# gaspachoo/EEG2Video

Measured on AMD Instinct MI355X. Metric: 6-frame 288x512 clips/sec (50-step DDIM), higher is better.
Workload: dtype f32; 1 GPU; 1xMI355X: batch=8/GPU synthetic latents [B,4,6,36,64] + [B,77,768] cond, 50-step DDIM, CFG 12.5, 288x512x6 VAE decode, fp32 (BASELINE configs[1]); clips_per_gpu=8, ddim_steps=50, unet_samples_per_ddim_step=16, weights=random-init SD-v1-4 architecture, counter RNG seed 42/43, collective=none

## Files before the change

### eeg2video_amd/csrc/attn.hip

```cpp
#include "h16.h"
#include "kernels.h"
#include "prof.h"
#include "runtime.h"
#include "act_io.h"

#include <cstdlib>
#include <type_traits>

namespace e2v {

typedef float f32x16 __attribute__((ext_vector_type(16)));
typedef float f32x4 __attribute__((ext_vector_type(4)));

struct AttnBlock { int qb, head, sf; bool valid; };
__host__ __device__ __forceinline__ int attn_xcd_unit(const int n, const int F, const int heads) {
    return n % 8 == 0 ? 0 : (n * F) % 8 == 0 ? 1 : 2;
}
__device__ __forceinline__ AttnBlock attn_block_of(const AttnArgs& p, const int nqb) {
    const int b = blockIdx.x, xcd = b & 7, idx = b >> 3;
    const int S = p.n * p.F;
    const int unit = attn_xcd_unit(p.n, p.F, p.heads);
    AttnBlock r;
    if (unit == 0) {
        const int per = p.F * p.heads * nqb;
        const int ul = idx / per, w = idx - ul * per;
        const int smp = ul * 8 + xcd;
        const int f = w / (p.heads * nqb), w2 = w - f * (p.heads * nqb);
        r.sf = smp * p.F + f; r.head = w2 / nqb; r.qb = w2 - r.head * nqb; r.valid = smp < p.n;
    } else if (unit == 1) {
        const int per = p.heads * nqb;
        const int ul = idx / per, w = idx - ul * per;
        r.sf = ul * 8 + xcd; r.head = w / nqb; r.qb = w - r.head * nqb; r.valid = r.sf < S;
    } else {
        const int ul = idx / nqb;
        const int pair = ul * 8 + xcd;
        r.qb = idx - ul * nqb; r.sf = pair / p.heads; r.head = pair - r.sf * p.heads; r.valid = pair < S * p.heads;
    }
    return r;
}
__device__ __forceinline__ AttnBlock attn_block(const AttnArgs& p) { return attn_block_of(p, (p.Nq + 127) / 128); }
static inline unsigned attn_grid_of(const AttnArgs& a, const unsigned nqb) {
    const int unit = attn_xcd_unit(a.n, a.F, a.heads);
    if (unit == 0) return 8u * (a.n / 8) * (unsigned)(a.F * a.heads) * nqb;
    if (unit == 1) return 8u * ((a.n * a.F) / 8) * (unsigned)a.heads * nqb;
    return 8u * ((a.n * a.F * a.heads + 7) / 8) * nqb;
}
static inline unsigned attn_grid(const AttnArgs& a) { return attn_grid_of(a, (a.Nq + 127) / 128); }

std::string attn_shape_tag(const AttnArgs& a) {
    return " D" + std::to_string(a.D) + " Nq" + std::to_string(a.Nq) + " Nk" + std::to_string(a.Nk) + " n" + std::to_string(a.n) + " F" + std::to_string(a.F) +
           " h" + std::to_string(a.heads);
}

template <int D>
__global__ __launch_bounds__(256) void flash_attn_kernel(const AttnArgs p) {
    constexpr int LD = D + 4;
    constexpr int TF = D / 32;
    constexpr bool VREM = (D - 32 * TF) == 8;
    constexpr int T = VREM ? TF : (D + 31) / 32;
    constexpr int TA = T > 0 ? T : 1;
    constexpr int G = D / 8;
    constexpr int DQ = D / 4;
    constexpr int KT = 32;
    constexpr int NF4 = KT * DQ;
    constexpr int LPT = (NF4 + 255) / 256;
    extern __shared__ __attribute__((aligned(16))) float smem[];

    const int tid = threadIdx.x;
    const int lane = tid & 63, wave = tid >> 6;
    const int j = lane & 31, h = lane >> 5;
    const AttnBlock blk = attn_block(p);
    if (!blk.valid) return;
    const int sf = blk.sf;
    const int smp = sf / p.F, f = sf - smp * p.F;
    const int head = blk.head;
    const int q0 = (blk.qb * 4 + wave) * 32;
    const bool active = q0 < p.Nq;

    int nseg = 1;
    size_t kvbase[2];
    if (p.mode == 0) {
        kvbase[0] = (size_t)(smp * p.F) * p.Nk;
        kvbase[1] = (size_t)(smp * p.F + (f > 0 ? f - 1 : 0)) * p.Nk;
        nseg = f >= 2 ? 2 : 1;
    } else {
        kvbase[0] = kvbase[1] = (size_t)smp * p.Nk;
    }
    const int tps = (p.Nk + KT - 1) / KT;
    const int ntiles = nseg * tps;

    f32x4 qf[G];
    {
        const int qrow = min(q0 + j, p.Nq - 1);
        const float* qp = p.q + ((size_t)sf * p.Nq + qrow) * p.ldq + head * D + h * 4;
        const float c = p.scale * 1.44269504088896340736f;
#pragma unroll
        for (int g = 0; g < G; ++g) {
            qf[g] = *reinterpret_cast<const f32x4*>(qp + g * 8);
            qf[g] *= c;
        }
    }

    constexpr unsigned OOB = 0x80000000u;
    auto rsrc_of = [](const void* ptr) {
        const unsigned long long v = reinterpret_cast<unsigned long long>(ptr);
        const unsigned lo = __builtin_amdgcn_readfirstlane((unsigned)v);
        const unsigned hi = __builtin_amdgcn_readfirstlane((unsigned)(v >> 32));
        return __builtin_amdgcn_make_buffer_rsrc(reinterpret_cast<void*>(((unsigned long long)hi << 32) | lo), (short)0, 0x7FFFFFF0,
                                                 0x00020000);
    };
    int ld_row[LPT];
    unsigned ld_off[LPT];
#pragma unroll
    for (int e = 0; e < LPT; ++e) {
        const int idx = tid + 256 * e;
        const int row = idx / DQ, c4 = idx - row * DQ;
        ld_row[e] = row;
        ld_off[e] = idx < NF4 ? (unsigned)(row * p.ldkv + c4 * 4) * 4u : OOB;
    }
    f32x4 kreg[LPT], vreg[LPT];
    auto load_tile = [&](int tt) {
        const int seg = tt / tps;
        const int key0 = (tt - seg * tps) * KT;
        const size_t first = (kvbase[seg] + key0) * p.ldkv + head * D;
        const __amdgpu_buffer_rsrc_t rk = rsrc_of(p.k + first), rv = rsrc_of(p.v + first);
        const int left = p.Nk - key0;
#pragma unroll
        for (int e = 0; e < LPT; ++e) {
            unsigned off = ld_off[e];
            if (left < KT) off = ld_row[e] < left ? off : OOB;
            kreg[e] = __builtin_bit_cast(f32x4, __builtin_amdgcn_raw_buffer_load_b128(rk, off, 0, 0));
            vreg[e] = __builtin_bit_cast(f32x4, __builtin_amdgcn_raw_buffer_load_b128(rv, off, 0, 0));
        }
    };
    auto store_tile = [&](int buf) {
        float* Ks = smem + buf * (2 * KT * LD);
        float* Vs = Ks + KT * LD;
#pragma unroll
        for (int e = 0; e < LPT; ++e) {
            const int idx = tid + 256 * e;
            if (idx < NF4) {
                const int row = idx / DQ, c4 = idx - row * DQ;
                *reinterpret_cast<f32x4*>(Ks + row * LD + c4 * 4) = kreg[e];
                *reinterpret_cast<f32x4*>(Vs + row * LD + c4 * 4) = vreg[e];
            }
        }
    };

    f32x16 acc[TA];
#pragma unroll
    for (int t = 0; t < TA; ++t)
#pragma unroll
        for (int r = 0; r < 16; ++r) acc[t][r] = 0.f;
    f32x4 rem0 = {0.f, 0.f, 0.f, 0.f}, rem1 = {0.f, 0.f, 0.f, 0.f};
    float m_i = -INFINITY, l_i = 0.f;

    load_tile(0);
    store_tile(0);
    __syncthreads();

    for (int tt = 0; tt < ntiles; ++tt) {
        const int buf = tt & 1;
        if (tt + 1 < ntiles) load_tile(tt + 1);
        const int seg_c = tt / tps;
        const int kbase = (tt - seg_c * tps) * KT;
        auto tile_body = [&](const int key0, const int sub, auto ragged) {
            const float* Ks = smem + buf * (2 * KT * LD) + sub * 32 * LD;
            const float* Vs = smem + buf * (2 * KT * LD) + KT * LD + sub * 32 * LD;
            const f32x16 zero16 = {0.f, 0.f, 0.f, 0.f, 0.f, 0.f, 0.f, 0.f, 0.f, 0.f, 0.f, 0.f, 0.f, 0.f, 0.f, 0.f};
            f32x16 st;
            const float* kp = Ks + j * LD + h * 4;
#pragma unroll
            for (int g = 0; g < G; ++g) {
                const f32x4 kf = *reinterpret_cast<const f32x4*>(kp + g * 8);
#pragma unroll
                for (int s = 0; s < 4; ++s)
                    st = __builtin_amdgcn_mfma_f32_32x32x2f32(kf[s], qf[g][s], (g == 0 && s == 0) ? zero16 : st, 0, 0, 0);
            }
            if constexpr (decltype(ragged)::value) {
#pragma unroll
                for (int r = 0; r < 16; ++r) {
                    const int key = key0 + (r & 3) + 8 * (r >> 2) + 4 * h;
                    if (key >= p.Nk) st[r] = -INFINITY;
                }
            }
            float mt = st[0];
#pragma unroll
            for (int r = 1; r < 16; ++r) mt = __builtin_fmaxf(mt, st[r]);
            mt = __builtin_fmaxf(mt, __shfl_xor(mt, 32));
            const float m_new = __builtin_fmaxf(m_i, mt);
            const bool moved = __any(m_new > m_i);
            float ps = 0.f;
#pragma unroll
            for (int r = 0; r < 16; ++r) {
                st[r] = __builtin_amdgcn_exp2f(st[r] - m_new);
                ps += st[r];
            }
            float alpha = 1.0f;
            if (moved) {
                alpha = __builtin_amdgcn_exp2f(m_i - m_new);
                l_i *= alpha;
            }
            l_i += ps;
            m_i = m_new;
#pragma unroll
            for (int t = 0; t < T; ++t) {
                if (moved) {
#pragma unroll
                    for (int r = 0; r < 16; ++r) acc[t][r] *= alpha;
                }
                const int dv = min(t * 32 + j, D - 1);
                const float* vp = Vs + (4 * h) * LD + dv;
#pragma unroll
                for (int r = 0; r < 16; ++r) {
                    const float vv = vp[((r & 3) + 8 * (r >> 2)) * LD];
                    acc[t] = __builtin_amdgcn_mfma_f32_32x32x2f32(vv, st[r], acc[t], 0, 0, 0);
                }
            }
            if constexpr (VREM) {
                if (moved) {
                    rem0 *= alpha;
                    rem1 *= alpha;
                }
                const float* vr = Vs + (4 * h) * LD + 32 * TF;
#pragma unroll
                for (int r = 0; r < 16; ++r) {
                    const float* row = vr + ((r & 3) + 8 * (r >> 2)) * LD;
                    const f32x4 v0 = *reinterpret_cast<const f32x4*>(row);
                    const f32x4 v1 = *reinterpret_cast<const f32x4*>(row + 4);
                    rem0 += v0 * st[r];
                    rem1 += v1 * st[r];
                }
            }
        };
#pragma unroll
        for (int sub = 0; sub < KT / 32; ++sub) {
            const int key0 = kbase + 32 * sub;
            if (active && key0 < p.Nk) {
                if (key0 + 32 <= p.Nk) tile_body(key0, sub, std::false_type{});
                else tile_body(key0, sub, std::true_type{});
            }
        }
        if (tt + 1 < ntiles) store_tile(buf ^ 1);
        __syncthreads();
    }

    const float l_tot = l_i + __shfl_xor(l_i, 32);
    if constexpr (VREM) {
#pragma unroll
        for (int e = 0; e < 4; ++e) {
            rem0[e] += __shfl_xor(rem0[e], 32);
            rem1[e] += __shfl_xor(rem1[e], 32);
        }
    }
    if (active && q0 + j < p.Nq) {
        const float inv = 1.0f / l_tot;
        float* op = p.o + ((size_t)sf * p.Nq + q0 + j) * p.ldo + head * D;
#pragma unroll
        for (int t = 0; t < T; ++t)
#pragma unroll
            for (int rg = 0; rg < 4; ++rg) {
                const int dv = t * 32 + 8 * rg + 4 * h;
                if (dv < D) {
                    f32x4 o;
#pragma unroll
                    for (int e = 0; e < 4; ++e) o[e] = acc[t][rg * 4 + e] * inv;
                    *reinterpret_cast<f32x4*>(op + dv) = o;
                }
            }
        if constexpr (VREM) {
            const f32x4 o = (h ? rem1 : rem0) * inv;
            *reinterpret_cast<f32x4*>(op + 32 * TF + 4 * h) = o;
        }
    }
}

typedef __bf16 abf16x4 __attribute__((ext_vector_type(4)));
typedef __bf16 abf16x8 __attribute__((ext_vector_type(8)));

template <typename H, int D, bool FOLD, int KT>
__global__ __launch_bounds__(256) void flash_attn_b16io_kernel(const AttnArgs p) {
    constexpr int DP = (D + 15) / 16 * 16;
    constexpr int KS = DP / 16;
    constexpr int T = (D + 31) / 32;
    constexpr int KROW = DP * 2 + 16;
    constexpr int VROW = ((T * 16) % 32 == 16) ? T * 64 : T * 64 + 64;
    constexpr int KBYTES = KT * KROW, VBYTES = KT * VROW;
    constexpr int STAGE = (KBYTES + VBYTES + 15) / 16 * 16;
    constexpr bool SUMV = (D % 32) != 0;
    constexpr int LROW = D % 32, LREG = 4 * (LROW / 8) + (LROW & 3), LHALF = (LROW >> 2) & 1;
    constexpr int C8 = D / 8;
    constexpr int NP = KT * C8;
    constexpr int LPT = (NP + 255) / 256;
    extern __shared__ __attribute__((aligned(16))) char smem_h[];

    const int tid = threadIdx.x;
    const int lane = tid & 63, wave = tid >> 6;
    const int j = lane & 31, h = lane >> 5;
    const AttnBlock blk = attn_block(p);
    if (!blk.valid) return;
    const int sf = blk.sf;
    const int smp = sf / p.F, f = sf - smp * p.F;
    const int head = blk.head;
    const int q0 = (blk.qb * 4 + wave) * 32;
    const bool active = q0 < p.Nq;
    const H* __restrict__ Q = reinterpret_cast<const H*>(p.q);
    const H* __restrict__ K = reinterpret_cast<const H*>(p.k);
    const H* __restrict__ V = reinterpret_cast<const H*>(p.v);

    int nseg = 1;
    size_t kvbase[2];
    if (p.mode == 0) {
        kvbase[0] = (size_t)(smp * p.F) * p.Nk;
        kvbase[1] = (size_t)(smp * p.F + (f > 0 ? f - 1 : 0)) * p.Nk;
        nseg = f >= 2 ? 2 : 1;
    } else {
        kvbase[0] = kvbase[1] = (size_t)smp * p.Nk;
    }
    const int tps = (p.Nk + KT - 1) / KT;
    const int ntiles = nseg * tps;

    for (int i = tid * 16; i < 2 * STAGE; i += 256 * 16)
        *reinterpret_cast<f32x4*>(smem_h + i) = f32x4{0.f, 0.f, 0.f, 0.f};
    if constexpr (SUMV) {
        __syncthreads();
        if (tid < 2 * KT)
            *reinterpret_cast<H*>(smem_h + (tid / KT) * STAGE + KBYTES + (tid % KT) * VROW + D * 2) = (H)1.0f;
    }

    hx8<H> qf[KS];
    {
        const int qrow = min(q0 + j, p.Nq - 1);
        const H* qp = Q + ((size_t)sf * p.Nq + qrow) * p.ldq + head * D;
#pragma unroll
        for (int s = 0; s < KS; ++s) {
            const int k0 = 16 * s + 8 * h;
            hx8<H> a;
#pragma unroll
            for (int e = 0; e < 8; ++e) a[e] = (H)0.f;
            if (k0 < D) a = *reinterpret_cast<const hx8<H>*>(qp + k0);
            if constexpr (FOLD) {
                const float qs = p.scale * 1.44269504088896340736f;
#pragma unroll
                for (int e = 0; e < 8; ++e) a[e] = (H)((float)a[e] * qs);
            }
            qf[s] = a;
        }
    }
    const float sc = p.scale * 1.44269504088896340736f;
    __syncthreads();

    constexpr unsigned OOB = 0x80000000u;
    auto rsrc_of = [](const void* ptr) {
        const unsigned long long v = reinterpret_cast<unsigned long long>(ptr);
        const unsigned lo = __builtin_amdgcn_readfirstlane((unsigned)v);
        const unsigned hi = __builtin_amdgcn_readfirstlane((unsigned)(v >> 32));
        return __builtin_amdgcn_make_buffer_rsrc(reinterpret_cast<void*>(((unsigned long long)hi << 32) | lo), (short)0, 0x7FFFFFF0,
                                                 0x00020000);
    };
    int ld_row[LPT], ld_c8[LPT];
    unsigned ld_off[LPT];
#pragma unroll
    for (int e = 0; e < LPT; ++e) {
        const int idx = tid + 256 * e;
        const int row = idx / C8, c8 = idx - row * C8;
        ld_row[e] = row; ld_c8[e] = c8;
        ld_off[e] = idx < NP ? (unsigned)(row * p.ldkv + c8 * 8) * 2u : OOB;
    }
    f32x4 kreg[LPT], vreg[LPT];
    auto load_tile = [&](const int seg, const int key0) {
        const size_t first = (kvbase[seg] + key0) * p.ldkv + head * D;
        const __amdgpu_buffer_rsrc_t rk = rsrc_of(K + first), rv = rsrc_of(V + first);
        const int left = p.Nk - key0;
#pragma unroll
        for (int e = 0; e < LPT; ++e) {
            unsigned off = ld_off[e];
            if (left < KT) off = ld_row[e] < left ? off : OOB;
            kreg[e] = __builtin_bit_cast(f32x4, __builtin_amdgcn_raw_buffer_load_b128(rk, off, 0, 0));
            vreg[e] = __builtin_bit_cast(f32x4, __builtin_amdgcn_raw_buffer_load_b128(rv, off, 0, 0));
        }
    };
    auto store_tile = [&](int buf) {
        char* Kl = smem_h + buf * STAGE;
        char* Vl = Kl + KBYTES;
#pragma unroll
        for (int e = 0; e < LPT; ++e) {
            if (tid + 256 * e < NP) {
                *reinterpret_cast<f32x4*>(Kl + ld_row[e] * KROW + ld_c8[e] * 16) = kreg[e];
                *reinterpret_cast<f32x4*>(Vl + ld_row[e] * VROW + ld_c8[e] * 16) = vreg[e];
            }
        }
    };

    f32x16 acc[T];
#pragma unroll
    for (int t = 0; t < T; ++t)
#pragma unroll
        for (int r = 0; r < 16; ++r) acc[t][r] = 0.f;
// ... 495 lines not shown
                for (int x = 0; x < 4; ++x) {
                    unsigned v1, v2, v3;
                    split3(vreg[e][x], v1, v2, v3);
                    char* vd = Vl + (c4 * 4 + x) * VROW + row * 2;
                    *reinterpret_cast<unsigned short*>(vd) = (unsigned short)(v1 >> 16);
                    *reinterpret_cast<unsigned short*>(vd + VBYTES) = (unsigned short)(v2 >> 16);
                    *reinterpret_cast<unsigned short*>(vd + 2 * VBYTES) = (unsigned short)(v3 >> 16);
                }
            }
        }
    };

    f32x16 acc[T];
#pragma unroll
    for (int t = 0; t < T; ++t)
#pragma unroll
        for (int r = 0; r < 16; ++r) acc[t][r] = 0.f;
    float m_i = -INFINITY, l_i = 0.f;

    load_tile(0);
    store_tile(0);
    __syncthreads();

    constexpr int TA[6] = {1, 2, 0, 1, 0, 0}, TB[6] = {1, 0, 2, 0, 1, 0};
    for (int tt = 0; tt < ntiles; ++tt) {
        const int buf = tt & 1;
        if (tt + 1 < ntiles) load_tile(tt + 1);
        const int seg_c = tt / tps;
        const int key0 = (tt - seg_c * tps) * 32;
        if (active) {
            const char* Kl = smem_x + buf * STAGE;
            const char* Vl = Kl + 3 * KBYTES;
            f32x16 st;
#pragma unroll
            for (int r = 0; r < 16; ++r) st[r] = 0.f;
            const char* kp = Kl + j * KROW + h * 16;
#pragma unroll
            for (int s = 0; s < KS; ++s) {
                abf16x8 kf[3];
#pragma unroll
                for (int pl = 0; pl < 3; ++pl) kf[pl] = *reinterpret_cast<const abf16x8*>(kp + pl * KBYTES + s * 32);
#pragma unroll
                for (int t6 = 0; t6 < 6; ++t6)
                    st = __builtin_amdgcn_mfma_f32_32x32x16_bf16(kf[TA[t6]], __builtin_bit_cast(abf16x8, qf[TB[t6]][s]), st, 0, 0, 0);
            }
            if (key0 + 32 > p.Nk) {
#pragma unroll
                for (int r = 0; r < 16; ++r) {
                    const int key = key0 + (r & 3) + 8 * (r >> 2) + 4 * h;
                    if (key >= p.Nk) st[r] = -INFINITY;
                }
            }
            float mt = st[0];
#pragma unroll
            for (int r = 1; r < 16; ++r) mt = __builtin_fmaxf(mt, st[r]);
            mt = __builtin_fmaxf(mt, __shfl_xor(mt, 32));
            const float m_new = __builtin_fmaxf(m_i, mt);
            const bool moved = __any(m_new > m_i);
            float ps = 0.f;
#pragma unroll
            for (int r = 0; r < 16; ++r) {
                st[r] = __builtin_amdgcn_exp2f(st[r] - m_new);
                ps += st[r];
            }
            float alpha = 1.0f;
            if (moved) {
                alpha = __builtin_amdgcn_exp2f(m_i - m_new);
                l_i *= alpha;
            }
            l_i += ps;
            m_i = m_new;
            au32x4 pf[3][2];
#pragma unroll
            for (int s = 0; s < 2; ++s)
#pragma unroll
                for (int e = 0; e < 4; ++e) {
                    unsigned a1, a2, a3, b1, b2, b3;
                    split3(st[8 * s + 2 * e], a1, a2, a3);
                    split3(st[8 * s + 2 * e + 1], b1, b2, b3);
                    pf[0][s][e] = (a1 >> 16) | (b1 & 0xFFFF0000u);
                    pf[1][s][e] = (a2 >> 16) | (b2 & 0xFFFF0000u);
                    pf[2][s][e] = (a3 >> 16) | (b3 & 0xFFFF0000u);
                }
#pragma unroll
            for (int t = 0; t < T; ++t) {
                if (moved) {
#pragma unroll
                    for (int r = 0; r < 16; ++r) acc[t][r] *= alpha;
                }
                const char* vrow = Vl + min(t * 32 + j, D - 1) * VROW + h * 8;
#pragma unroll
                for (int s = 0; s < 2; ++s) {
                    abf16x8 vf[3];
#pragma unroll
                    for (int pl = 0; pl < 3; ++pl) {
                        const abf16x4 lo = *reinterpret_cast<const abf16x4*>(vrow + pl * VBYTES + s * 32);
                        const abf16x4 hi = *reinterpret_cast<const abf16x4*>(vrow + pl * VBYTES + s * 32 + 16);
                        vf[pl] = __builtin_shufflevector(lo, hi, 0, 1, 2, 3, 4, 5, 6, 7);
                    }
#pragma unroll
                    for (int t6 = 0; t6 < 6; ++t6)
                        acc[t] = __builtin_amdgcn_mfma_f32_32x32x16_bf16(vf[TA[t6]], __builtin_bit_cast(abf16x8, pf[TB[t6]][s]), acc[t], 0, 0, 0);
                }
            }
        }
        if (tt + 1 < ntiles) store_tile(buf ^ 1);
        __syncthreads();
    }

    const float l_tot = l_i + __shfl_xor(l_i, 32);
    if (active && q0 + j < p.Nq) {
        const float inv = 1.0f / l_tot;
        float* op = p.o + ((size_t)sf * p.Nq + q0 + j) * p.ldo + head * D;
#pragma unroll
        for (int t = 0; t < T; ++t)
#pragma unroll
            for (int rg = 0; rg < 4; ++rg) {
                const int dv = t * 32 + 8 * rg + 4 * h;
                if (dv < D) {
                    f32x4 o;
#pragma unroll
                    for (int e = 0; e < 4; ++e) o[e] = acc[t][rg * 4 + e] * inv;
                    *reinterpret_cast<f32x4*>(op + dv) = o;
                }
            }
    }
}
template <int D>
static void launch_flash_x3(const AttnArgs& a, hipStream_t s) {
    constexpr int DP = (D + 15) / 16 * 16;
    constexpr size_t stage = ((size_t)3 * (32 * (DP * 2 + 16) + ((D + 31) / 32) * 32 * 72) + 15) / 16 * 16;
    constexpr size_t smem = 2 * stage;
    E2V_KATTR(&flash_attn_x3_kernel<D>, smem);
    dim3 grid(attn_grid(a), 1, 1);
    const double nk = a.mode == 0 ? 2.0 * a.Nk : (double)a.Nk;
    const double probs = (double)a.n * a.F * a.heads;
    ProfScope ps(a.mode == 0 ? "flash_attn_f32x3_sparse_causal" : "flash_attn_f32x3_cross", 4.0 * probs * a.Nq * nk * D,
                 4.0 * probs * D * (2.0 * a.Nq + 2.0 * (a.mode == 0 ? a.Nk : (double)a.Nk / a.F)), s);
    E2V_KLAUNCH((flash_attn_x3_kernel<D>), grid, dim3(256), smem, s, a);
}

template <int D>
static void launch_flash(const AttnArgs& a, hipStream_t s) {
    constexpr size_t smem = (size_t)2 * 2 * 32 * (D + 4) * sizeof(float);
    E2V_KATTR(&flash_attn_kernel<D>, smem);
    dim3 grid(attn_grid(a), 1, 1);
    const double nk = a.mode == 0 ? 2.0 * a.Nk : (double)a.Nk;
    const double probs = (double)a.n * a.F * a.heads;
    std::string pname = a.mode == 0 ? "flash_attn_sparse_causal" : "flash_attn_cross";
    if (prof_detail()) pname += attn_shape_tag(a);
    ProfScope ps(pname.c_str(), 4.0 * probs * a.Nq * nk * D,
                 4.0 * probs * D * (2.0 * a.Nq + 2.0 * (a.mode == 0 ? a.Nk : (double)a.Nk / a.F)), s);
    dry_tag(" -> flash_attn_kernel");
    E2V_KLAUNCH((flash_attn_kernel<D>), grid, dim3(256), smem, s, a);
}

bool flash_attention_supports(int D) {
    switch (D) {
        case 8: case 16: case 32: case 40: case 64: case 80: case 160: return true;
        default: return false;
    }
}

void flash_attention(const AttnArgs& a, hipStream_t s) {
    if (!flash_attention_supports(a.D))
        throw Error(E2V_EINVAL, "attention head dim " + std::to_string(a.D) + " has no kernel instance (supported: 8, 16, 32, 40, 64, 80, 160)");
    if (a.io_bf16) {
        if ((a.ldq | a.ldkv | a.ldo) & 7) throw Error(E2V_ESHAPE, "bf16 attention: row strides must be multiples of 8 elements");
        switch (a.D) {
            case 8: launch_flash_b16io<8>(a, s); return;
            case 16: launch_flash_b16io<16>(a, s); return;
            case 32: launch_flash_b16io<32>(a, s); return;
            case 40: launch_flash_b16io<40>(a, s); return;
            case 64: launch_flash_b16io<64>(a, s); return;
            case 80: launch_flash_b16io<80>(a, s); return;
            default: launch_flash_b16io<160>(a, s); return;
        }
    }
    if (a.x3) {
        switch (a.D) {
            case 8: launch_flash_x3<8>(a, s); return;
            case 16: launch_flash_x3<16>(a, s); return;
            case 32: launch_flash_x3<32>(a, s); return;
            case 40: launch_flash_x3<40>(a, s); return;
            case 64: launch_flash_x3<64>(a, s); return;
            case 80: launch_flash_x3<80>(a, s); return;
            default: launch_flash_x3<160>(a, s); return;
        }
    }
    switch (a.D) {
        case 8: launch_flash<8>(a, s); break;
        case 16: launch_flash<16>(a, s); break;
        case 32: launch_flash<32>(a, s); break;
        case 40: launch_flash<40>(a, s); break;
        case 64: launch_flash<64>(a, s); break;
        case 80: launch_flash<80>(a, s); break;
        default: launch_flash<160>(a, s); break;
    }
}

static constexpr int FMAX = 8;
template <typename T>
__global__ __launch_bounds__(256) void temporal_attn_kernel(const T* __restrict__ qkv, int ld, T* __restrict__ out,
                                                            int ldo, int n, int F, int HW, int heads, int D, float scale) {
    const size_t total = (size_t)n * HW * heads * F;
    const size_t gid = blockIdx.x * (size_t)blockDim.x + threadIdx.x;
    if (gid >= total) return;
    const int i = gid % F;
    const int head = (gid / F) % heads;
    const size_t ph = gid / ((size_t)F * heads);
    const int pix = ph % HW;
    const int smp = ph / HW;
    const int C = heads * D;
    const size_t row0 = (size_t)smp * F * HW + pix;
    const T* qp = qkv + (row0 + (size_t)i * HW) * ld + head * D;
    const T* kp = qkv + row0 * ld + C + head * D;
    const T* vp = qkv + row0 * ld + 2 * C + head * D;
    const size_t fstride = (size_t)HW * ld;
    float s[FMAX];
#pragma unroll
    for (int jf = 0; jf < FMAX; ++jf) s[jf] = 0.f;
    for (int c = 0; c < D; c += 4) {
        const f32x4 qv = ld4(qp + c);
#pragma unroll
        for (int jf = 0; jf < FMAX; ++jf)
            if (jf < F) {
                const f32x4 kv = ld4(kp + jf * fstride + c);
                s[jf] += qv[0] * kv[0] + qv[1] * kv[1] + qv[2] * kv[2] + qv[3] * kv[3];
            }
    }
    float m = -INFINITY;
#pragma unroll
    for (int jf = 0; jf < FMAX; ++jf)
        if (jf < F) {
            s[jf] *= scale;
            m = fmaxf(m, s[jf]);
        }
    float l = 0.f;
#pragma unroll
    for (int jf = 0; jf < FMAX; ++jf)
        if (jf < F) {
            s[jf] = expf(s[jf] - m);
            l += s[jf];
        }
    const float inv = 1.0f / l;
    T* op = out + (row0 + (size_t)i * HW) * ldo + head * D;
    for (int c = 0; c < D; c += 4) {
        f32x4 o = {0.f, 0.f, 0.f, 0.f};
#pragma unroll
        for (int jf = 0; jf < FMAX; ++jf)
            if (jf < F) {
                const f32x4 vv = ld4(vp + jf * fstride + c);
                o += vv * (s[jf] * inv);
            }
        st4(op + c, o);
    }
}

template <typename T>
__global__ __launch_bounds__(128) void temporal_attn_lds_kernel(const T* __restrict__ qkv, int ld, T* __restrict__ out,
                                                                int ldo, int F, int HW, int C, int D, float scale, int PB,
                                                                int CS, int npg) {
    extern __shared__ __attribute__((aligned(16))) float sm[];
    const int smp = blockIdx.x / npg, p0 = (blockIdx.x - smp * npg) * PB;
    const int c_base = blockIdx.y * CS;
    if constexpr (!std::is_same<T, float>::value) {
        const int CO = CS / 8;
        const int total = F * PB * 3 * CO;
        for (int idx = threadIdx.x; idx < total; idx += 128) {
            const int c8 = idx % CO;
            int r = idx / CO;
            const int part = r % 3; r /= 3;
            const int pp = r % PB;
            const int f = r / PB;
            const int pix = p0 + pp;
            f32x4 lo = {0.f, 0.f, 0.f, 0.f}, hi = lo;
            if (pix < HW) {
                const hx8<T> v = *reinterpret_cast<const hx8<T>*>(qkv + ((size_t)(smp * F + f) * HW + pix) * ld + part * C + c_base + c8 * 8);
#pragma unroll
                for (int e = 0; e < 4; ++e) { lo[e] = (float)v[e]; hi[e] = (float)v[4 + e]; }
            }
            *reinterpret_cast<f32x4*>(sm + (size_t)idx * 8) = lo;
            *reinterpret_cast<f32x4*>(sm + (size_t)idx * 8 + 4) = hi;
        }
    } else {
        const int CQ = CS / 4;
        const int total = F * PB * 3 * CQ;
        for (int idx = threadIdx.x; idx < total; idx += 128) {
            const int c4 = idx % CQ;
            int r = idx / CQ;
            const int part = r % 3; r /= 3;
            const int pp = r % PB;
            const int f = r / PB;
            const int pix = p0 + pp;
            f32x4 v = {0.f, 0.f, 0.f, 0.f};
            if (pix < HW) v = ld4(qkv + ((size_t)(smp * F + f) * HW + pix) * ld + part * C + c_base + c4 * 4);
            *reinterpret_cast<f32x4*>(sm + (size_t)idx * 4) = v;
        }
    }
    __syncthreads();
    const int hs = CS / D;
    const int items = PB * hs * F;
    for (int item = threadIdx.x; item < items; item += 128) {
        const int i = item % F;
        const int hh = (item / F) % hs;
        const int pp = item / (F * hs);
// ... 495 lines not shown
```

### eeg2video_amd/csrc/bgemm.hip

```cpp
#include "igemm_epi.h"
#include "prof.h"
#include "runtime.h"

#include <cstdio>
#include <cstdlib>
#include <string>

#include <map>
#include <mutex>

namespace e2v {

static std::mutex& knob_mutex() { static std::mutex m; return m; }
static std::map<std::string, int>& knob_table() { static std::map<std::string, int> t; return t; }
int* knob(const char* name, int dflt) {
    std::lock_guard<std::mutex> lk(knob_mutex());
    auto& t = knob_table();
    auto it = t.find(name);
    if (it == t.end()) {
        const char* e = std::getenv(name);
        it = t.emplace(name, e ? std::atoi(e) : dflt).first;
    }
    return &it->second;
}
bool set_knob(const char* name, int value) {
    std::lock_guard<std::mutex> lk(knob_mutex());
    auto& t = knob_table();
    auto it = t.find(name);
    if (it == t.end()) {
        static const char* const known[] = {"E2V_BGEMM_PERS", "E2V_BGEMM_256LIN", "E2V_BGEMM_256", "E2V_BGEMM_T256", "E2V_BGEMM_T256P", "E2V_BGEMM_T256P_BIAS_LDS",
                                            "E2V_ATTN_KT64", "E2V_ATTN_Q64", "E2V_ATTN_CROSS_RESIDENT", "E2V_TATTN_WAVE", "E2V_LN_ROWS", "E2V_BGEMM_UP2X",
                                            "E2V_SPLITK", "E2V_SPLITK_FORCE", "E2V_GN_FUSED_SMALL", "E2V_BGEMM_S3_SMALL", "E2V_SMALL_FAMILY_CLIPS", "E2V_POOL_GUARD"
#ifdef E2V_AB
                                            , "E2V_BGEMM_S3", "E2V_BGEMM_LIN", "E2V_BGEMM_T256_TAIL", "E2V_ATTN_FOLD", "E2V_ATTN_Q64P", "E2V_ATTN_Q64_NW", "E2V_GN_ROWS", "E2V_GN_GROUP_MB", "E2V_GN_SKIP_PARTIAL", "E2V_GN_RB", "E2V_GN_RB_EPILOGUE",
                                            "E2V_BGEMM_256_MINROUNDS", "E2V_BGEMM_T256_MINK", "E2V_BGEMM_T256_MINTILES", "E2V_BGEMM_T256P_MAXK", "E2V_BGEMM_T256P_MINTILES", "E2V_GN_CHUNK_ROWS",
                                            "E2V_GN_CHUNK_ROWS_SMALL", "E2V_IGEMM_HALF_BELOW", "E2V_SPLITK_MIN_DEPTH", "E2V_SPLITK_MAX_TILES", "E2V_GN_COOP", "E2V_LN_STATS_ONLY"
#endif
#ifdef E2V_ABLATE
                                            , "E2V_BGEMM_ABLATE"
#endif
        };
        bool ok = false;
        for (const char* k : known) ok = ok || std::string(k) == name;
        if (!ok) return false;
        it = t.emplace(name, value).first;
    }
    it->second = value;
    return true;
}

int pool_guard_kib() {
    static const int* const kib = knob("E2V_POOL_GUARD", 0);
    return *kib > 0 ? *kib : 0;
}

template <class F, int... T>
__device__ __forceinline__ void static_for_taps(F&& f, std::integer_sequence<int, T...>) {
    (f(std::integral_constant<int, T>{}), ...);
}

template <typename H, int BM, int BN, int WGM, int WGN, int STAGE = 128 * 128 * 2, bool LIN = false, int NST = 2, int CALLER = 0>
__device__ __forceinline__ void bgemm_tile(const IgemmArgs& p, const int rbg, const int n0, char* smem) {
    constexpr int BKE = 64;
    constexpr int ROWB = 128;
    constexpr int NW = WGM * WGN, NT = 64 * NW;
    constexpr int WM = BM / WGM, WN = BN / WGN;
    constexpr int TM = WM / 32, TN = WN / 32;
    constexpr int A_BYTES = BM * ROWB, B_BYTES = BN * ROWB;
    constexpr int APW = BM / 8 / NW, BPW = BN / 8 / NW;
    static_assert(APW >= 1 && BPW >= 1 && A_BYTES + B_BYTES <= STAGE, "tile does not fit the stage");
    const int z = p.batch > 1 ? rbg / p.nbm_per : 0;
    const int bm = rbg - z * p.nbm_per;

    const int tid = threadIdx.x;
    const int lane = tid & 63;
    const int wave = __builtin_amdgcn_readfirstlane(tid >> 6);
    const int wm = wave / WGN, wn = wave % WGN;

    const H* __restrict__ a0 = reinterpret_cast<const H*>(p.a0) + (size_t)z * p.sa0;
    const H* __restrict__ a1 = reinterpret_cast<const H*>(p.a1);
    const char* __restrict__ w = reinterpret_cast<const char*>(p.w16) + ((size_t)z * p.sw + (size_t)n0 * p.ldw) * 2;

    const int steps0 = (p.c0 + BKE - 1) / BKE, steps1 = (p.c1 + BKE - 1) / BKE;
    const int nk = p.taps * (steps0 + steps1);

    unsigned* tab = reinterpret_cast<unsigned*>(smem + NST * STAGE);
    const int hw_out = p.Ho * p.Wo, hw_in = p.Hs * p.Ws;
    const int img0 = p.taps == 1 ? 0 : (bm * BM) / hw_out;
    const size_t row_base = p.taps == 1 ? (size_t)bm * BM : (size_t)img0 * hw_in;
    for (int e = tid; !LIN && e < p.taps * BM; e += NT) {
        const int tap = e / BM, row = e - tap * BM;
        const int m = bm * BM + row;
        unsigned pix = ~0u;
        if (m < p.M) {
            if (p.taps == 1) {
                pix = (unsigned)row;
            } else {
                const int img = m / hw_out;
                const int rem = m - img * hw_out;
                const int oy = rem / p.Wo, ox = rem - oy * p.Wo;
                const int ky = (tap * 11) >> 5, kx = tap - 3 * ky;
                const int iy = oy * p.stride - p.pad + ky, ix = ox * p.stride - p.pad + kx;
                if ((unsigned)iy < (unsigned)p.Hi && (unsigned)ix < (unsigned)p.Wi) {
                    int sy = iy, sx = ix;
                    if (p.upsample) {
                        sy = min((int)floorf((float)iy * p.ups_h), p.Hs - 1);
                        sx = min((int)floorf((float)ix * p.ups_w), p.Ws - 1);
                    }
                    pix = (unsigned)(((img - img0) * p.Hs + sy) * p.Ws + sx);
                }
            }
        }
        tab[e] = pix;
    }
    constexpr unsigned OOB = 0x80000000u;
    const H* const a0b = a0 + row_base * p.lda0;
    const H* const a1b = p.c1 > 0 ? a1 + row_base * p.lda1 : a0b;
    const int a_records = (p.ablate & 2) ? 0 : 0x7FFFFFF0;
    auto rsrc_of = [](const void* ptr, const int records = 0x7FFFFFF0) {
        const unsigned long long v = reinterpret_cast<unsigned long long>(ptr);
        const unsigned lo = __builtin_amdgcn_readfirstlane((unsigned)v);
        const unsigned hi = __builtin_amdgcn_readfirstlane((unsigned)(v >> 32));
        return __builtin_amdgcn_make_buffer_rsrc(reinterpret_cast<void*>(((unsigned long long)hi << 32) | lo), (short)0, records,
                                                 0x00020000);
    };
    const __amdgpu_buffer_rsrc_t rw = rsrc_of(w);

    const int r8 = lane >> 3, pp = lane & 7;
    int a_row[APW];
    unsigned a_kc[APW];
#pragma unroll
    for (int i = 0; i < APW; ++i) {
        a_row[i] = 8 * (wave * APW + i) + r8;
        a_kc[i] = (unsigned)(pp ^ ((a_row[i] >> 1) & 7));
    }
    unsigned b_off[BPW], b_kc[BPW];
#pragma unroll
    for (int j = 0; j < BPW; ++j) {
        const int r = 8 * (wave * BPW + j) + r8;
        b_kc[j] = (unsigned)(pp ^ ((r >> 1) & 7));
        b_off[j] = (n0 + r < p.N) ? (unsigned)(r * p.ldw * 2) + b_kc[j] * 16u : OOB;
    }
    unsigned a_voff0[APW], a_voff1[APW];
#pragma unroll
    for (int i = 0; i < APW; ++i) {
        const bool in = bm * BM + a_row[i] < p.M;
        a_voff0[i] = in ? (unsigned)(a_row[i] * p.lda0 * 2) + a_kc[i] * 16u : OOB;
        a_voff1[i] = in ? (unsigned)(a_row[i] * p.lda1 * 2) + a_kc[i] * 16u : OOB;
    }
    if constexpr (!LIN) __syncthreads();

    int k_src = 0, k_cb = 0, k_tap = 0, cseg = p.c0, ldb = p.lda0 * 2;
    bool done = false;
    unsigned pixn[APW];
    if constexpr (!LIN) {
#pragma unroll
        for (int i = 0; i < APW; ++i) pixn[i] = tab[a_row[i]];
    }
    typedef __attribute__((address_space(3))) void* lds_ptr;
    auto issue = [&](const int buf) {
        char* Ab = smem + buf * STAGE;
        char* Bb = Ab + A_BYTES;
        if constexpr (LIN) {
            if (!done) {
                const unsigned so = (unsigned)k_cb * 2u;
                const unsigned sob = (unsigned)((k_src ? p.c0 : 0) + k_cb) * 2u;
                const bool whole = k_cb + BKE <= cseg;
                const __amdgpu_buffer_rsrc_t rsa = rsrc_of(k_src ? a1b : a0b, a_records);
#pragma unroll
                for (int i = 0; i < APW; ++i) {
                    const unsigned vo = k_src ? a_voff1[i] : a_voff0[i];
                    const unsigned off = (whole || k_cb + (int)a_kc[i] * 8 < cseg) ? vo : OOB;
                    __builtin_amdgcn_raw_ptr_buffer_load_lds(rsa, (lds_ptr)(Ab + (wave * APW + i) * 1024), 16, off, so, 0, 0);
                }
#pragma unroll
                for (int j = 0; j < BPW; ++j) {
                    const unsigned off = (whole || k_cb + (int)b_kc[j] * 8 < cseg) ? b_off[j] : OOB;
                    __builtin_amdgcn_raw_ptr_buffer_load_lds(rw, (lds_ptr)(Bb + (wave * BPW + j) * 1024), 16, off, sob, 0, 0);
                }
                k_cb += BKE;
                if (k_cb >= cseg) {
                    if (k_src == 0 && p.c1 > 0) { k_src = 1; k_cb = 0; cseg = p.c1; }
                    else done = true;
                }
            }
            return;
        }
// ... 899 lines not shown
```

Baseline: 0.5942 clips/s.

## Fold running max into QK MFMA accumulator init in f32 flash attention

The f32 flash-attention kernel now seeds the QK^T MFMA accumulator with the negated running max, so scores arrive already offset. Rescaling happens only when the tile max exceeds zero, and the cross-half max reduction uses v_permlane32_swap instead of a shuffle. It also unrolls the tile loop by two so the LDS buffer index is a compile-time constant, accumulates l in a 2-wide vector, and software-pipelines the V-remainder loads. The aim is to cut VALU subtract, max and shuffle work per tile, at the cost of more complex control flow and slightly different rounding.

Measured after the change: 0.5970 clips/s (median of 6 runs). Within noise of the previous version (+0.5%).

```diff
diff --git a/eeg2video_amd/csrc/attn.hip b/eeg2video_amd/csrc/attn.hip
--- a/eeg2video_amd/csrc/attn.hip
+++ b/eeg2video_amd/csrc/attn.hip
@@ -52,7 +52,9 @@
            " h" + std::to_string(a.heads);
 }
 
-template <int D>
+typedef float f32x2 __attribute__((ext_vector_type(2)));
+
+template <int D, bool FOLD = true>
 __global__ __launch_bounds__(256) void flash_attn_kernel(const AttnArgs p) {
     constexpr int LD = D + 4;
     constexpr int TF = D / 32;
@@ -153,40 +155,105 @@
 #pragma unroll
         for (int r = 0; r < 16; ++r) acc[t][r] = 0.f;
     f32x4 rem0 = {0.f, 0.f, 0.f, 0.f}, rem1 = {0.f, 0.f, 0.f, 0.f};
-    float m_i = -INFINITY, l_i = 0.f;
+    float m_i = FOLD ? 0.f : -INFINITY, l_i = 0.f;
+    f32x2 l2 = {0.f, 0.f};
 
     load_tile(0);
     store_tile(0);
     __syncthreads();
 
-    for (int tt = 0; tt < ntiles; ++tt) {
-        const int buf = tt & 1;
-        if (tt + 1 < ntiles) load_tile(tt + 1);
-        const int seg_c = tt / tps;
-        const int kbase = (tt - seg_c * tps) * KT;
-        auto tile_body = [&](const int key0, const int sub, auto ragged) {
-            const float* Ks = smem + buf * (2 * KT * LD) + sub * 32 * LD;
-            const float* Vs = smem + buf * (2 * KT * LD) + KT * LD + sub * 32 * LD;
-            const f32x16 zero16 = {0.f, 0.f, 0.f, 0.f, 0.f, 0.f, 0.f, 0.f, 0.f, 0.f, 0.f, 0.f, 0.f, 0.f, 0.f, 0.f};
-            f32x16 st;
-            const float* kp = Ks + j * LD + h * 4;
-#pragma unroll
-            for (int g = 0; g < G; ++g) {
-                const f32x4 kf = *reinterpret_cast<const f32x4*>(kp + g * 8);
-#pragma unroll
-                for (int s = 0; s < 4; ++s)
-                    st = __builtin_amdgcn_mfma_f32_32x32x2f32(kf[s], qf[g][s], (g == 0 && s == 0) ? zero16 : st, 0, 0, 0);
-            }
-            if constexpr (decltype(ragged)::value) {
-#pragma unroll
-                for (int r = 0; r < 16; ++r) {
-                    const int key = key0 + (r & 3) + 8 * (r >> 2) + 4 * h;
-                    if (key >= p.Nk) st[r] = -INFINITY;
-                }
-            }
-            float mt = st[0];
-#pragma unroll
-            for (int r = 1; r < 16; ++r) mt = __builtin_fmaxf(mt, st[r]);
+    auto tile_body = [&](const int key0, auto bufc, auto ragged, const bool first) {
+        const int buf = bufc;
+        const float* Ks = smem + buf * (2 * KT * LD);
+        const float* Vs = smem + buf * (2 * KT * LD) + KT * LD;
+        const f32x16 zero16 = {0.f, 0.f, 0.f, 0.f, 0.f, 0.f, 0.f, 0.f, 0.f, 0.f, 0.f, 0.f, 0.f, 0.f, 0.f, 0.f};
+        f32x16 st, negm;
+        if constexpr (FOLD) {
+            const f32x2 nm = {-m_i, -m_i};
+            negm = __builtin_shufflevector(nm, nm, 0, 1, 0, 1, 0, 1, 0, 1, 0, 1, 0, 1, 0, 1, 0, 1);
+        }
+        const float* kp = Ks + j * LD + h * 4;
+#pragma unroll
+        for (int g = 0; g < G; ++g) {
+            const f32x4 kf = *reinterpret_cast<const f32x4*>(kp + g * 8);
+#pragma unroll
+            for (int s = 0; s < 4; ++s)
+                st = __builtin_amdgcn_mfma_f32_32x32x2f32(kf[s], qf[g][s], (g == 0 && s == 0) ? (FOLD ? negm : zero16) : st, 0, 0, 0);
+        }
+        const float* vr = Vs + (4 * h) * LD + 32 * TF;
+        auto rem_row = [&](const int r) { return vr + ((r & 3) + 8 * (r >> 2)) * LD; };
+        constexpr int RB = 2;
+        f32x4 rv0[RB], rv1[RB];
+        auto rem_load = [&](const int r0) {
+#pragma unroll
+            for (int e = 0; e < RB; ++e) {
+                rv0[e] = *reinterpret_cast<const f32x4*>(rem_row(r0 + e));
+                rv1[e] = *reinterpret_cast<const f32x4*>(rem_row(r0 + e) + 4);
+            }
+        };
+        auto rem_fma = [&](const int r0) {
+#pragma unroll
+            for (int e = 0; e < RB; ++e) {
+                rem0 += rv0[e] * st[r0 + e];
+                rem1 += rv1[e] * st[r0 + e];
+            }
+        };
+        if constexpr (decltype(ragged)::value) {
+#pragma unroll
+            for (int r = 0; r < 16; ++r) {
+                const int key = key0 + (r & 3) + 8 * (r >> 2) + 4 * h;
+                if (key >= p.Nk) st[r] = -INFINITY;
+            }
+        }
+        float mt = st[0];
+#pragma unroll
+        for (int r = 1; r < 16; ++r) mt = __builtin_fmaxf(mt, st[r]);
+        if constexpr (FOLD) {
+            auto finish = [&]() {
+                if constexpr (VREM) rem_load(0);
+#pragma unroll
+                for (int r = 0; r < 16; ++r) st[r] = __builtin_amdgcn_exp2f(st[r]);
+#pragma unroll
+                for (int r = 0; r < 16; r += 2) l2 += f32x2{st[r], st[r + 1]};
+#pragma unroll
+                for (int t = 0; t < T; ++t) {
+                    const int dv = min(t * 32 + j, D - 1);
+                    const float* vp = Vs + (4 * h) * LD + dv;
+#pragma unroll
+                    for (int r = 0; r < 16; ++r) {
+                        const float vv = vp[((r & 3) + 8 * (r >> 2)) * LD];
+                        acc[t] = __builtin_amdgcn_mfma_f32_32x32x2f32(vv, st[r], acc[t], 0, 0, 0);
+                    }
+                }
+                if constexpr (VREM) {
+#pragma unroll
+                    for (int r0 = 0; r0 < 16; r0 += RB) {
+                        rem_fma(r0);
+                        if (r0 + RB < 16) rem_load(r0 + RB);
+                    }
+                }
+            };
+            {
+                float a = mt, b = mt;
+                asm volatile("s_nop 1\n\tv_permlane32_swap_b32 %0, %1" : "+v"(a), "+v"(b));
+                mt = __builtin_fmaxf(a, b);
+            }
+            const float d = first ? mt : __builtin_fmaxf(mt, 0.f);
+            const float alpha = first ? 1.0f : __builtin_amdgcn_exp2f(-d);
+            if (first || __any(mt > 0.f)) {
+                asm volatile("; maximum moved" ::: "memory");
+#pragma unroll
+                for (int r = 0; r < 16; ++r) st[r] -= d;
+            }
+            m_i = first ? d : m_i + d;
+            l2 *= alpha;
+#pragma unroll
+            for (int t = 0; t < T; ++t)
+#pragma unroll
+                for (int r = 0; r < 16; ++r) acc[t][r] *= alpha;
+            if constexpr (VREM) { rem0 *= alpha; rem1 *= alpha; }
+            finish();
+        } else {
             mt = __builtin_fmaxf(mt, __shfl_xor(mt, 32));
             const float m_new = __builtin_fmaxf(m_i, mt);
             const bool moved = __any(m_new > m_i);
@@ -222,28 +289,33 @@
                     rem0 *= alpha;
                     rem1 *= alpha;
                 }
-                const float* vr = Vs + (4 * h) * LD + 32 * TF;
 #pragma unroll
                 for (int r = 0; r < 16; ++r) {
-                    const float* row = vr + ((r & 3) + 8 * (r >> 2)) * LD;
-                    const f32x4 v0 = *reinterpret_cast<const f32x4*>(row);
-                    const f32x4 v1 = *reinterpret_cast<const f32x4*>(row + 4);
+                    const f32x4 v0 = *reinterpret_cast<const f32x4*>(rem_row(r));
+                    const f32x4 v1 = *reinterpret_cast<const f32x4*>(rem_row(r) + 4);
                     rem0 += v0 * st[r];
                     rem1 += v1 * st[r];
                 }
             }
-        };
-#pragma unroll
-        for (int sub = 0; sub < KT / 32; ++sub) {
-            const int key0 = kbase + 32 * sub;
-            if (active && key0 < p.Nk) {
-                if (key0 + 32 <= p.Nk) tile_body(key0, sub, std::false_type{});
-                else tile_body(key0, sub, std::true_type{});
-            }
+        }
+    };
+    auto step = [&](const int tt, auto bufc) {
+        const int buf = bufc;
+        if (tt + 1 < ntiles) load_tile(tt + 1);
+        const int seg_c = tt / tps;
+        const int key0 = (tt - seg_c * tps) * KT;
+        if (active) {
+            if (key0 + 32 <= p.Nk) tile_body(key0, bufc, std::false_type{}, tt == 0);
+            else tile_body(key0, bufc, std::true_type{}, tt == 0);
         }
         if (tt + 1 < ntiles) store_tile(buf ^ 1);
         __syncthreads();
-    }
+    };
+    for (int tt = 0; tt < ntiles; tt += 2) {
+        step(tt, std::integral_constant<int, 0>{});
+        if (tt + 1 < ntiles) step(tt + 1, std::integral_constant<int, 1>{});
+    }
+    if constexpr (FOLD) l_i = l2[0] + l2[1];
 
     const float l_tot = l_i + __shfl_xor(l_i, 32);
     if constexpr (VREM) {
@@ -1045,6 +1117,14 @@
     ProfScope ps(pname.c_str(), 4.0 * probs * a.Nq * nk * D,
                  4.0 * probs * D * (2.0 * a.Nq + 2.0 * (a.mode == 0 ? a.Nk : (double)a.Nk / a.F)), s);
     dry_tag(" -> flash_attn_kernel");
+#ifdef E2V_AB
+    static const int* const fold = knob("E2V_ATTN_F32_FOLD", 1);
+    if (!*fold) {
+        E2V_KATTR((&flash_attn_kernel<D, false>), smem);
+        E2V_KLAUNCH((flash_attn_kernel<D, false>), grid, dim3(256), smem, s, a);
+        return;
+    }
+#endif
     E2V_KLAUNCH((flash_attn_kernel<D>), grid, dim3(256), smem, s, a);
 }
 
diff --git a/eeg2video_amd/csrc/bgemm.hip b/eeg2video_amd/csrc/bgemm.hip
--- a/eeg2video_amd/csrc/bgemm.hip
+++ b/eeg2video_amd/csrc/bgemm.hip
@@ -32,7 +32,7 @@
                                             "E2V_ATTN_KT64", "E2V_ATTN_Q64", "E2V_ATTN_CROSS_RESIDENT", "E2V_TATTN_WAVE", "E2V_LN_ROWS", "E2V_BGEMM_UP2X",
                                             "E2V_SPLITK", "E2V_SPLITK_FORCE", "E2V_GN_FUSED_SMALL", "E2V_BGEMM_S3_SMALL", "E2V_SMALL_FAMILY_CLIPS", "E2V_POOL_GUARD"
 #ifdef E2V_AB
-                                            , "E2V_BGEMM_S3", "E2V_BGEMM_LIN", "E2V_BGEMM_T256_TAIL", "E2V_ATTN_FOLD", "E2V_ATTN_Q64P", "E2V_ATTN_Q64_NW", "E2V_GN_ROWS", "E2V_GN_GROUP_MB", "E2V_GN_SKIP_PARTIAL", "E2V_GN_RB", "E2V_GN_RB_EPILOGUE",
+                                            , "E2V_BGEMM_S3", "E2V_BGEMM_LIN", "E2V_BGEMM_T256_TAIL", "E2V_ATTN_FOLD", "E2V_ATTN_F32_FOLD", "E2V_ATTN_Q64P", "E2V_ATTN_Q64_NW", "E2V_GN_ROWS", "E2V_GN_GROUP_MB", "E2V_GN_SKIP_PARTIAL", "E2V_GN_RB", "E2V_GN_RB_EPILOGUE",
                                             "E2V_BGEMM_256_MINROUNDS", "E2V_BGEMM_T256_MINK", "E2V_BGEMM_T256_MINTILES", "E2V_BGEMM_T256P_MAXK", "E2V_BGEMM_T256P_MINTILES", "E2V_GN_CHUNK_ROWS",
                                             "E2V_GN_CHUNK_ROWS_SMALL", "E2V_IGEMM_HALF_BELOW", "E2V_SPLITK_MIN_DEPTH", "E2V_SPLITK_MAX_TILES", "E2V_GN_COOP", "E2V_LN_STATS_ONLY"
 #endif
```
